# JuliaGaussianProcesses/ApproximateGPs.jl

Measured on AMD Instinct MI355X. Metric: SVGP ELBO evals/sec at N=1e6, M=1024, higher is better.
Workload: dtype f64

## Files before the change

### approximategps.jl_amd/csrc/api.hip

```cpp
#include <hip/hip_runtime.h>

#include <algorithm>
#include <functional>
#include <memory>
#include <cmath>
#include <cstdio>
#include <cstddef>
#include <cstdlib>
#include <cstring>
#include <new>
#include <string>
#include <vector>

#include "../../include/svgp_mi355x.h"
#include "ctx.hpp"
#include "kernels.hpp"
#include "knobs.hpp"
#include "lik.hpp"

using namespace svgp;

inline unsigned event_flags(bool timing) {
  static const bool fence = exp_int("SVGP_EVENT_FENCE", 0) == 1;
  return (timing ? 0u : unsigned(hipEventDisableTiming)) | (fence ? 0u : unsigned(hipEventDisableSystemFence));
// ... 161 lines not shown
KernelParams kparams(const svgp_model* m) {
  KernelParams kp;
  kp.family = m->desc.kernel;
  kp.d = m->d;
  kp.variance = m->desc.variance;
  kp.invl = m->invl.p;
  return kp;
}

inline size_t info_bytes(int64_t Mp) { return (sizeof(int) * size_t(1 + 2 * (Mp / 128)) + 255) / 256 * 256; }
int ensure_overlap(svgp_ctx* ctx, size_t state_doubles);
int enqueue_prep(svgp_ctx* ctx, svgp_model* m, bool overlap = false, const RowHook* hook = nullptr) {
  hipStream_t s = ctx->stream;
  const KernelParams kp = kparams(m);
  HIPC(ctx, hipMemsetAsync(m->info.as<int>(), 0, info_bytes(m->Mp), s));
  launch_scale_inputs(m->dtype, s, m->z_raw.p, m->desc.layout_z, m->d, m->M, m->Mp, m->invl.p, m->zs.p);
  KCHECK(ctx, "scale_inputs");
  if (overlap) {
    launch_pack_q(m->dtype, s, m->Lq_raw.p, m->m_raw.p, m->M, m->Mp, m->U.p, m->mp.p);
    KCHECK(ctx, "pack_q");
    HIPC(ctx, hipEventRecord(ctx->ev_fork, s));
    TREC(ctx, ctx->ev_ov[0], s);
    if (hook && hook->fn) hook->fn(hook->user, -1);
  }
  launch_kuu(m->dtype, s, kp, m->zs.p, m->M, m->Mp, m->desc.jitter, m->L.p);
  KCHECK(ctx, "kuu");
  TREC(ctx, ctx->ev_chol[0], s);
  hipEvent_t rows[16] = {};
  if (overlap) std::copy(std::begin(ctx->ev_row), std::end(ctx->ev_row), rows);
  launch_potrf(m->dtype, s, m->L.p, m->T.p, m->Mp, m->info.as<int>(), reinterpret_cast<unsigned*>(m->info.as<int>() + 1), ctx->num_cus, overlap ? rows : nullptr,
               overlap ? hook : nullptr);
// ... 93 lines not shown
  StripPlan plan = strip_plan(m->dtype, m->Mp, len, ctx->num_cus);
  if (plan.concurrent_tail && (o.A || o.C || o.At || o.Ct)) plan = strip_plan_single(m->dtype, m->Mp, len, ctx->num_cus);
  const size_t wb_main = plan.grid ? strip_work_bytes(m->dtype, m->Mp, plan.nt, plan.grid) : 0;
  const size_t wb_tail = plan.nt_tail ? strip_work_bytes(m->dtype, m->Mp, plan.nt_tail, plan.grid_tail) : 0;
  int rc = ensure_scratch(ctx, plan.concurrent_tail ? wb_main : (wb_main > wb_tail ? wb_main : wb_tail), size_t(len));
  if (rc) return rc;
  if (plan.concurrent_tail) {
    rc = ensure_stream2(ctx);
    if (rc) return rc;
    rc = ctx->work2.reserve(ctx, wb_tail, "the concurrent tail's scratch");
    if (rc) return rc;
  }
  StripArgs a{};
  a.T = m->T.p;
  a.U = m->U.p;
  a.zs = m->zs.p;
  a.mp = m->mp.p;
  a.x = x;
  a.work = ctx->work.p;
  a.counter = ctx->counter.as<unsigned>();
  a.mom_mu = ctx->mom_mu();
  a.mom_var = ctx->mom_var();
  a.A_out = o.A;
  a.C_out = o.C;
  a.At_out = o.At;
  a.Ct_out = o.Ct;
  a.lda = o.lda;
  a.ldx = ldx;
  a.off = off;
  a.len = len;
  a.Mp = m->Mp;
// ... 117 lines not shown

void seg_row_hook(void* user, int row) {
  SegRun& r = *static_cast<SegRun*>(user);
  if (r.rc == SVGP_OK) r.rc = seg_enqueue_row(r, row);
}

int seg_prepare_forward(svgp_ctx* ctx, svgp_model* m, const void* x, int64_t ldx, int64_t off, int64_t len, const OverlapPlan& op, SegRun& r) {
  const int nP = int(m->Mp / 128);
  const size_t wb1 = strip_work_bytes(m->dtype, m->Mp, op.nt, int(op.nstrips)), wb = wb1;
  int rc = ctx->work_seg.reserve(ctx, wb, "the segmented strips' scratch");
  if (rc == SVGP_OK) rc = ensure_scratch(ctx, 0, size_t(len));
  if (rc) return rc;
  r.ctx = ctx; r.m = m; r.op = op; r.grad = false; r.nP = nP; r.wb1 = wb1;
  r.split = seg_split_factor(ctx, nP, op.nstrips);
  StripArgs& a = r.a;
  a.T = m->T.p; a.U = m->U.p; a.zs = m->zs.p; a.mp = m->mp.p; a.x = x; a.work = ctx->work_seg.p; a.counter = ctx->counter2.as<unsigned>();
  a.mom_mu = ctx->mom_mu(); a.mom_var = ctx->mom_var();
  a.ldx = ldx; a.off = off; a.len = len; a.Mp = m->Mp; a.M = m->M; a.kp = kparams(m); a.mean_const = m->desc.mean_const;
  a.seg_state = ctx->seg_state.as<double>();
  return SVGP_OK;
}

int seg_finish_forward(svgp_ctx* ctx, svgp_model* m, const void* y, int64_t off, int64_t len, const StripOuts& o, SegRun& r) {
  hipStream_t s = ctx->stream, s2 = ctx->stream2;
  if (r.rc) return r.rc;
  int launches = r.nP + 1;
  if (r.split > 1) {
    StripArgs& a = r.a;
    const int rcs = seg_split_setup(ctx, a, r.split, r.op.nstrips);
    if (rcs) return rcs;
    a.seg_lo = a.seg_hi = r.nP;
// ... 360 lines not shown
  if (!out) return fail(ctx, SVGP_INVALID_ARG, "null out pointer");
  *out = nullptr;
  int rc = validate_desc(ctx, desc);
  if (rc) return rc;
  HIPC(ctx, hipSetDevice(ctx->device));
  svgp_model* m = new (std::nothrow) svgp_model();
  if (!m) return SVGP_OOM;
  m->M = desc->M;
  m->Mp = (desc->M + 127) / 128 * 128;
  m->dtype = desc->dtype;
  m->d = desc->d;
  m->es = esize(desc->dtype);
  const size_t es = m->es, M = size_t(m->M), Mp = size_t(m->Mp);
  struct { DevBuf* b; size_t bytes; } allocs[] = {
      {&m->z_raw, M * m->d * es}, {&m->m_raw, M * es},     {&m->Lq_raw, M * M * es}, {&m->invl, size_t(m->d) * es},
      {&m->zs, Mp * m->d * es},   {&m->L, Mp * Mp * es},   {&m->T, Mp * Mp * es},    {&m->U, Mp * Mp * es},
      {&m->mp, Mp * es},          {&m->scal, (8 + Mp) * sizeof(double)},             {&m->info, info_bytes(Mp)},
      {&m->B, desc->parametrization == SVGP_CENTERED ? Mp * Mp * es : 0},
  };
  for (auto& a : allocs)
    if (a.bytes && a.b->alloc(a.bytes) != hipSuccess) {
      svgp_model_free(ctx, m);
      return alloc_failed(ctx, "for model buffers");
    }
  if (hipMemsetAsync(m->T.p, 0, Mp * Mp * es, ctx->stream) != hipSuccess) {
    svgp_model_free(ctx, m);
    return fail(ctx, SVGP_HIP_ERROR, "hipMemsetAsync failed for the model's T buffer");
  }
  rc = upload_params(ctx, m, desc);
  if (rc) {
    svgp_model_free(ctx, m);
    return rc;
// ... 110 lines not shown
  if (rc == SVGP_OK) rc = svgp_elbo(ctx, m, D, 0, n, num_data, elbo_out, terms_out);
  else if (ctx->comm) rc = elbo_collective(ctx, rc);
  svgp_data_free(ctx, D);
  svgp_model_free(ctx, m);
  return rc;
}

int32_t svgp_kuf(svgp_ctx* ctx, svgp_model* m, const svgp_data* data, int64_t off, int64_t len, void* Kuf_out_host) {
  int rc = check_batch(ctx, m, data, off, len, false);
  if (rc) return rc;
  HIPC(ctx, hipSetDevice(ctx->device));
  hipStream_t s = ctx->stream;
  const size_t bytes = size_t(m->M) * size_t(len) * m->es;
  rc = ctx->kuf_buf.reserve(ctx, bytes, "Kuf");
  if (rc) return rc;
  launch_scale_inputs(m->dtype, s, m->z_raw.p, m->desc.layout_z, m->d, m->M, m->Mp, m->invl.p, m->zs.p);
  TREC(ctx, ctx->ev[0], s);
  launch_kuf(m->dtype, s, kparams(m), m->zs.p, m->M, m->Mp, data->x.p, data->ldx, off, len, ctx->kuf_buf.p);
  TREC(ctx, ctx->ev[1], s);
  HIPC(ctx, hipGetLastError());
  if (Kuf_out_host) HIPC(ctx, hipMemcpyAsync(Kuf_out_host, ctx->kuf_buf.p, bytes, hipMemcpyDeviceToHost, s));
  HIPC(ctx, hipStreamSynchronize(s));
  float t = 0;
  (void)elapsed_ms(ctx, &t, ctx->ev[0], ctx->ev[1]);
  ctx->timing = svgp_timing{};
  ctx->timing.ms_kuf = t;
  ctx->timing.ms_total = t;
  return SVGP_OK;
}

int32_t svgp_posterior(svgp_ctx* ctx, svgp_model* m, void* Lk_out, void* alpha_out, void* B_out) {
// ... 299 lines not shown
    if (rc) return rc;
    ext_gmu = ctx->ext_g.as<double>();
    ext_gv = ext_gmu + ctx->ext_g.cap / 16;
    HIPC(ctx, hipMemcpyAsync(ext_gmu, gc.ext_gmu, size_t(len) * 8, hipMemcpyHostToDevice, s));
    HIPC(ctx, hipMemcpyAsync(ext_gv, gc.ext_gv, size_t(len) * 8, hipMemcpyHostToDevice, s));
  }
  const bool uniform_w = m->desc.likelihood == SVGP_LIK_GAUSSIAN && !gc.ext_gmu && m->gh_n == 0 && ctx->kn.syrk_uniform;
  static const int early_knob = exp_int("SVGP_SYRK_EARLY", 1);
  const bool syrk_early = gop.on && uniform_w && early_knob != 0;
  if (syrk_early) {
    rc = w->Gmm.reserve(ctx, size_t(std::min<int64_t>(Mp / 128, w->nslices)) * size_t(Mp) * size_t(Mp) * m->es, "the gradient workspace");
    if (rc) return rc;
  }
  auto strip_args = [&](int64_t c0, int64_t clen, LikParams& lpc) -> StripArgs {
    StripArgs a{};
    a.T = m->T.p; a.U = m->U.p; a.zs = m->zs.p; a.mp = m->mp.p; a.x = data->x.p; a.work = ctx->work.p; a.counter = ctx->counter.as<unsigned>();
    a.At_out = w->At.p; a.ldx = data->ldx; a.off = off + c0; a.len = clen; a.Mp = Mp; a.M = M; a.kp = kp;
    a.mean_const = m->desc.mean_const;
    if (gc.mux) a.mux = static_cast<const char*>(gc.mux) + size_t(c0) * es;
    a.mom_mu = ctx->mom_mu(); a.mom_var = ctx->mom_var();
    a.R = w->Rcm.p; a.alpha = w->alpha.p; a.Pt_out = w->Pt.p;
    lpc = lp;
    if (gc.ext_gmu) { lpc.lik = kLikExternal; lpc.gh_x = ext_gmu + c0; lpc.gh_w = ext_gv + c0; }
    return a;
  };
  const void* Bq = centered ? m->B.p : w->Lqp.p;
  auto grad_pre_chain = [&](hipStream_t st) -> int {
    HIPC(ctx, hipMemsetAsync(w->zero_blk.p, 0, w->zero_b, st));
    launch_setvec_f64(st, w->invl_d.as<double>(), m->invl_host.data(), m->d);
    if (!centered) launch_pad_lower(dt, st, m->Lq_raw.p, M, Mp, w->Lqp.p);
    gemm_mm(ctx, w, dt, st, Bq, Bq, Mp, w->G2.p, kMmXUp | kMmYUp);
// ... 812 lines not shown
    int nt, grid; int64_t nstrips;
    chunk_plan(clen, nt, grid, nstrips);
    wb_max = std::max(wb_max, strip_work_bytes(dt, Mp, nt, grid));
  }
  rc = ensure_scratch(ctx, wb_max, size_t(nc));
  if (rc) return rc;
  double* bpart = c->bpart.as<double>();
  double* spart = c->spart.as<double>();
  double* scal = c->scal.as<double>();
  for (int64_t c0 = 0; c0 < len; c0 += nc) {
    const int64_t clen = (len - c0 < nc) ? len - c0 : nc;
    const int64_t ncp = (clen + 127) / 128 * 128;
    int nt, grid; int64_t nstrips;
    chunk_plan(clen, nt, grid, nstrips);
    StripArgs a{};
    a.T = m->T.p; a.zs = m->zs.p; a.x = data->x.p; a.work = ctx->work.p; a.counter = ctx->counter.as<unsigned>();
    a.At_out = w->At.p; a.ldx = data->ldx; a.off = off + c0; a.len = clen; a.Mp = Mp; a.M = M; a.kp = kparams(m);
    a.mom_var = ctx->mom_var();
    HIPC(ctx, hipMemsetAsync(a.counter, 0, sizeof(unsigned), s));
    launch_trsm_point_major(dt, s, a, nt, grid, nstrips);
    KCHECK(ctx, "strip (phase 1, point-major A)");
    const int64_t n16 = (clen + 15) / 16 * 16;
    if (n16 > clen) HIPC(ctx, hipMemsetAsync(static_cast<char*>(w->At.p) + size_t(clen) * size_t(Mp) * es, 0, size_t(n16 - clen) * size_t(Mp) * es, s));
    const int64_t sl = ((ncp + ns_syrk - 1) / ns_syrk + 15) / 16 * 16;
    launch_syrk_uniform(dt, s, w->At.p, 1.0, 1.0, nullptr, 0.0, 1.0, Mp, n16, sl, ns_syrk, w->G1.p, c0 == 0 ? 1 : 0);
    KCHECK(ctx, "syrk (C = A A')");
    launch_collapsed_reduce(dt, s, w->At.p, data->y.p, a.mom_var, Mp, off + c0, clen, m->desc.mean_const, c0 == 0 ? 1 : 0, bpart, spart);
    KCHECK(ctx, "collapsed reduce (b, rr, t)");
  }
  const double sigma2 = m->desc.lik_sigma2;
  int* info_b = c->info_b.as<int>();
// ... 347 lines not shown
```

### approximategps.jl_amd/csrc/ctx.hpp

```cpp
#pragma once
#include <hip/hip_runtime.h>

#include <cstdlib>
#include <string>
#include <vector>

#include "../../include/svgp_mi355x.h"
#include "knobs.hpp"

namespace svgp {
inline int fail(svgp_ctx* ctx, int code, const std::string& msg);
inline int alloc_failed(svgp_ctx* ctx, const std::string& where);


struct DevBuf {
  void* p = nullptr;
  size_t cap = 0;
  bool own = true;
  DevBuf() = default;
  DevBuf(const DevBuf&) = delete;
  DevBuf& operator=(const DevBuf&) = delete;
  ~DevBuf() { release(); }
  void release() {
    if (p && own) (void)hipFree(p);
// ... 153 lines not shown
struct svgp_data {
  int dtype = 0, d = 0;
  int64_t n = 0, ldx = 0;
  svgp::DevBuf x;
  svgp::DevBuf y;
};

struct svgp_model {
  svgp_model_desc desc{};
  std::vector<double> invl_host;
  int64_t M = 0, Mp = 0;
  int dtype = 0, d = 0;
  size_t es = 8;
  svgp::DevBuf z_raw, m_raw, Lq_raw;
  svgp::DevBuf invl, zs, L, T, U, mp, B;
  svgp::DevBuf scal;
  svgp::DevBuf info;
  svgp::DevBuf gh_x, gh_w;
  int gh_n = 0;
  bool prepared = false;
  svgp::DevBuf mu_z;
  double kl = 0, logdet_kuu = 0;
  int chol_info = 0;
};

struct svgp_group {
  std::vector<svgp_ctx*> ctxs;
  std::string err;
};

// ... 44 lines not shown
```

### approximategps.jl_amd/csrc/kernels.hpp

```cpp
#pragma once
#include <hip/hip_runtime.h>
#include <stdint.h>

namespace svgp {

struct KernelParams {
  int family;
  int d;
  double variance;
  const void* invl;
};

constexpr int kLikExternal = -1;
struct LikParams {
  int lik;
  int gh_n;
  double sigma2;
  double digamma_alpha;
  const double* gh_x;
  const double* gh_w;
  int clamp_neg_var;
  double mean_const;
};

void launch_scale_inputs(int dtype, hipStream_t s, const void* z, int layout, int d, int64_t M, int64_t Mp,
                         const void* invl, void* zs);
void launch_transpose_colvecs(int dtype, hipStream_t s, const void* x_dn, int d, int64_t n, int64_t ldx, void* x_fm);
void launch_kuu(int dtype, hipStream_t s, const KernelParams& kp, const void* zs, int64_t M, int64_t Mp,
                double jitter, void* Kuu);
struct RowHook { void (*fn)(void* user, int row) = nullptr; void* user = nullptr; };
void launch_potrf(int dtype, hipStream_t s, void* A, void* T, int64_t Mp, int* info, unsigned* sync, int num_cus, hipEvent_t* row_events = nullptr,
                  const RowHook* hook = nullptr);
int potrf_max_row_events();
void launch_pack_q(int dtype, hipStream_t s, const void* Lq, const void* m, int64_t M, int64_t Mp, void* U, void* mp);
void launch_kl_terms(int dtype, hipStream_t s, const void* Lq, const void* m, const void* Lk, int64_t M, int64_t Mp,
                     double* scal);
void launch_pack_q_ld(int dtype, hipStream_t s, const void* Lq, int64_t ldq, const void* m, int64_t M, int64_t Mp, void* U,
                       void* mp);
void launch_kl_terms_ld(int dtype, hipStream_t s, const void* Lq, int64_t ldq, const void* m, const void* Lk, int64_t M,
                        int64_t Mp, double* scal);
void launch_trsv2(int dtype, hipStream_t s, const void* L, const void* Tm, int64_t Mp, int trans, void* x);
void launch_trsm_mat(int dtype, hipStream_t s, const void* Tm, int64_t Mp, void* X);
void launch_pad_lower(int dtype, hipStream_t s, const void* Lq, int64_t M, int64_t Mp, void* out);
void launch_shift_vec(int dtype, hipStream_t s, const void* m, double shift, int64_t M, int64_t Mp, void* out);
void launch_shift_sub_vec(int dtype, hipStream_t s, const void* m, double shift, const void* mu, int64_t M, int64_t Mp, void* out);
void launch_extract_lower(int dtype, hipStream_t s, const void* A, int64_t Mp, int64_t M, void* out);

enum : int { kSegPregen = 1, kSegPhase2 = 2, kSegLoad = 4, kSegStore = 8 };
struct StripArgs {
  const void* T;
  const void* U;
  const void* zs;
  const void* mp;
  const void* x;
  unsigned* counter;
  void* work;
  double* mom_mu;
  double* mom_var;
  void* A_out;
  void* C_out;
  void* At_out;
  void* Ct_out;
  int64_t lda;
  int64_t ldx, off, len;
  int64_t Mp, M;
  KernelParams kp;
  double mean_const;
// ... 109 lines not shown
```

### approximategps.jl_amd/csrc/prep.hip

```cpp
#define SVGP_DIAG_TU_PREP
#include "device_common.hpp"
#include "kernels.hpp"
#include "knobs.hpp"

#include <hip/hip_ext.h>
#include <cstdlib>
#include <algorithm>
#include <cmath>
#include <map>
#include <mutex>
#include <vector>

namespace svgp {
namespace {

template <typename T>
__global__ void scale_inputs_kernel(const T* __restrict__ z, int layout, int d, int64_t M, int64_t Mp,
                                    const T* __restrict__ invl, T* __restrict__ zs) {
  const int64_t i = int64_t(blockIdx.x) * blockDim.x + threadIdx.x;
  const int f = blockIdx.y;
  if (i >= Mp) return;
  T v = T(0);
  if (i < M) v = (layout == 1 ? z[int64_t(f) * M + i] : z[i * d + f]) * invl[f];
  zs[int64_t(f) * Mp + i] = v;
}

template <typename T>
__global__ void transpose_colvecs_kernel(const T* __restrict__ x, int d, int64_t n, int64_t ldx, T* __restrict__ out) {
  const int64_t i = int64_t(blockIdx.x) * blockDim.x + threadIdx.x;
  if (i >= n) return;
  for (int f = 0; f < d; ++f) out[int64_t(f) * ldx + i] = x[i * d + f];
}

template <typename T, int DREG>
__global__ void __launch_bounds__(k256) kuu_kernel(KernelParams kp, const T* __restrict__ zs, int64_t M, int64_t Mp, T jitter,
                                                   T* __restrict__ K) {
  constexpr int JB = 16;
  const int64_t i = int64_t(blockIdx.x) * k256 + threadIdx.x;
  const int64_t j0 = int64_t(blockIdx.y) * JB;
// ... 820 lines not shown
    hipLaunchKernelGGL((chol_tile_kernel<T, MODE_TRSM, CNT>), dim3((nP * (nP - 1) / 2) * NCH), dim3(k256), lds_tile, s, A, Tm, Mp, -1, 0, info, sync);
    dbg("T panels", s);
  }
}

}

std::string take_note_text() { return take_note(); }

#define SVGP_DISPATCH(dtype, expr_d, expr_f) \
  do {                                       \
    if ((dtype) == 0) { expr_d; } else { expr_f; } \
  } while (0)

void launch_scale_inputs(int dtype, hipStream_t s, const void* z, int layout, int d, int64_t M, int64_t Mp,
                         const void* invl, void* zs) {
  dim3 grid((unsigned)((Mp + 255) / 256), (unsigned)d);
  SVGP_DISPATCH(dtype,
                hipLaunchKernelGGL(scale_inputs_kernel<double>, grid, dim3(256), 0, s, (const double*)z, layout, d, M, Mp, (const double*)invl, (double*)zs),
                hipLaunchKernelGGL(scale_inputs_kernel<float>, grid, dim3(256), 0, s, (const float*)z, layout, d, M, Mp, (const float*)invl, (float*)zs));
}

void launch_transpose_colvecs(int dtype, hipStream_t s, const void* x, int d, int64_t n, int64_t ldx, void* out) {
  dim3 grid((unsigned)((n + 255) / 256));
  SVGP_DISPATCH(dtype,
                hipLaunchKernelGGL(transpose_colvecs_kernel<double>, grid, dim3(256), 0, s, (const double*)x, d, n, ldx, (double*)out),
                hipLaunchKernelGGL(transpose_colvecs_kernel<float>, grid, dim3(256), 0, s, (const float*)x, d, n, ldx, (float*)out));
}

void launch_kuu(int dtype, hipStream_t s, const KernelParams& kp, const void* zs, int64_t M, int64_t Mp, double jitter,
                void* Kuu) {
  dim3 grid((unsigned)((Mp + 255) / 256), (unsigned)(Mp / 16));
  if (kp.d <= 8) {
    SVGP_DISPATCH(dtype,
                  hipLaunchKernelGGL((kuu_kernel<double, 8>), grid, dim3(256), 0, s, kp, (const double*)zs, M, Mp, jitter, (double*)Kuu),
// ... 107 lines not shown
```

### approximategps.jl_amd/csrc/strip.hip

```cpp
#define SVGP_DIAG_TU_STRIP
#include "device_common.hpp"
#include "kernels.hpp"
#include "knobs.hpp"
#include "lik.hpp"

#ifndef SVGP_ASYNC
#define SVGP_ASYNC 1
#endif
#ifndef SVGP_TRI
#define SVGP_TRI 3
#endif

#include <cstdlib>
#include <type_traits>

namespace svgp {

namespace {

#ifndef SVGP_PREGEN_EXPTAB
#define SVGP_PREGEN_EXPTAB 1
#endif
template <typename T, int NT, int NTHR, int F, int DL>
__device__ __forceinline__ void pregen_mfma(const T* __restrict__ xs, const T* __restrict__ zs, int d, int64_t Mp, int64_t M,
                                            double variance_d, T* __restrict__ work, const double* __restrict__ exptab = nullptr) {
  constexpr int KS = DL / 4, JT = NT / 16, NW = NTHR / 64;
  constexpr bool XREG = (DL <= 16);
  using M16 = Mfma16<T>;
  using acc_t = typename M16::acc_t;
  const int lane = threadIdx.x & 63, wave = threadIdx.x >> 6, l15 = lane & 15, g = lane >> 4;
  const T variance = T(variance_d);
  const T c1 = (F == KSE) ? T(-0.5) : T(1);
  const T c0 = (F == KSE) ? T(log(variance_d)) : T(0);
  const T ascale = (F == KSE) ? T(1) : T(-2);
  T xb[XREG ? JT : 1][XREG ? KS : 1], xn[JT];
  const T* __restrict__ xl = xs + g * NT + l15;
#pragma unroll
  for (int jt = 0; jt < JT; ++jt) {
    T s = T(0);
// ... 55 lines not shown
#pragma unroll
        for (int r = 0; r < 4; ++r) work[(k0 + M16::row(lane, r)) * NT + jt * 16 + l15] = out[r];
      } else {
#pragma unroll
        for (int r = 0; r < 4; ++r) {
          const int64_t k = k0 + M16::row(lane, r);
          work[k * NT + jt * 16 + l15] = (k < M) ? out[r] : T(0);
        }
        asm volatile("" ::: "memory");
      }
    }
  }
}


template <typename G, typename T, int NT, int NTHR>
__device__ __forceinline__ void store_tile_point_major(const typename G::Acc& acc, T* __restrict__ smem, T* __restrict__ out,
                                                       int64_t c0, int64_t Mp, int row0) {
  constexpr int HC = NT < 64 ? NT : 64, RS = G::NB + (sizeof(T) == 8 ? 4 : 8), VEC = G::VEC, CPR = G::NB / VEC;
  using V = typename G::V;
  static_assert(size_t(HC) * RS * sizeof(T) <= ((SVGP_ASYNC && G::kAsync) ? G::ASYNC_LDS_BYTES : G::LDS_BYTES),
                "the transposition tile must fit the staging buffers");
#pragma unroll
  for (int p = 0; p < NT / HC; ++p) {
#pragma unroll
    for (int j = 0; j < G::NJ; ++j) {
      const int col = G::acc_col(j);
      if (col / HC == p) {
#pragma unroll
        for (int i = 0; i < G::MI; ++i)
// ... 37 lines not shown
__global__ void __launch_bounds__(NTHR, MINW) strip_kernel(StripArgs a, int64_t nstrips) {
  using G = TileGemm<T, NT, BK, NTHR, PAD>;
  using Acc = typename G::Acc;
  using QRegs = typename G::QRegs;
  constexpr int NB = G::NB, MI = G::MI, NJ = G::NJ, VEC = G::VEC;

  extern __shared__ __attribute__((aligned(16))) unsigned char smem_raw[];
  T* smem = reinterpret_cast<T*>(smem_raw);
  T* xs = smem;
  const int pre_dl = BIGD ? (a.kp.d <= 32 ? 32 : 64) : (a.kp.d <= 8 ? 8 : a.kp.d <= 16 ? 16 : 0);
  const int dl = pre_dl ? pre_dl : a.kp.d;

  const T* __restrict__ Tm = static_cast<const T*>(a.T);
  const T* __restrict__ U = static_cast<const T*>(a.U);
  const T* __restrict__ zs = static_cast<const T*>(a.zs);
  const T* __restrict__ mp = static_cast<const T*>(a.mp);
  const T* __restrict__ x = static_cast<const T*>(a.x);
  const T* __restrict__ invl = static_cast<const T*>(a.kp.invl);
  const int64_t Mp = a.Mp, M = a.M;
  const int d = a.kp.d, family = a.kp.family;
  const T variance = T(a.kp.variance);
  const int nP = int(Mp / NB);
  T* __restrict__ work = static_cast<T*>(a.work) + int64_t(blockIdx.x) * Mp * NT;
  T* __restrict__ workK = (GRAD && !diag::ablate<256>) ? static_cast<T*>(a.work) + (int64_t(gridDim.x) + blockIdx.x) * Mp * NT : work;
  const int tid = threadIdx.x, lane = tid & 63;
  const typename G::QOff qoff = G::q_offsets(NT);

  __shared__ unsigned next_strip;
#if SVGP_PREGEN_EXPTAB
  __shared__ double s_exptab[64];
// ... 45 lines not shown
            const V xf = *reinterpret_cast<const V*>(xs + f * NT + c);
#pragma unroll
            for (int q = 0; q < VEC; ++q) {
              const T df = xf[q] - zf;
              r2[q] = fma(df, df, r2[q]);
            }
          }
          V out;
#pragma unroll
          for (int q = 0; q < VEC; ++q) out[q] = (k < M) ? kappa<T>(F, r2[q], variance) : T(0);
          *reinterpret_cast<V*>(workK + int64_t(k) * NT + c) = out;
        }
      };
      if constexpr (BIGD) {
        if (pre_dl == 32) {
          if (family == KSE) pregen_mfma<T, NT, NTHR, KSE, 32>(xs, zs, d, Mp, M, a.kp.variance, workK, exptab);
          else if (family == KM32) pregen_mfma<T, NT, NTHR, KM32, 32>(xs, zs, d, Mp, M, a.kp.variance, workK);
          else pregen_mfma<T, NT, NTHR, KM52, 32>(xs, zs, d, Mp, M, a.kp.variance, workK);
        } else {
          if (family == KSE) pregen_mfma<T, NT, NTHR, KSE, 64>(xs, zs, d, Mp, M, a.kp.variance, workK, exptab);
          else if (family == KM32) pregen_mfma<T, NT, NTHR, KM32, 64>(xs, zs, d, Mp, M, a.kp.variance, workK);
          else pregen_mfma<T, NT, NTHR, KM52, 64>(xs, zs, d, Mp, M, a.kp.variance, workK);
        }
      } else if (pre_dl == 8) {
        if (family == KSE) pregen_mfma<T, NT, NTHR, KSE, 8>(xs, zs, d, Mp, M, a.kp.variance, workK, exptab);
        else if (family == KM32) pregen_mfma<T, NT, NTHR, KM32, 8>(xs, zs, d, Mp, M, a.kp.variance, workK);
        else pregen_mfma<T, NT, NTHR, KM52, 8>(xs, zs, d, Mp, M, a.kp.variance, workK);
      } else if (pre_dl == 16) {
        if (family == KSE) pregen_mfma<T, NT, NTHR, KSE, 16>(xs, zs, d, Mp, M, a.kp.variance, workK, exptab);
        else if (family == KM32) pregen_mfma<T, NT, NTHR, KM32, 16>(xs, zs, d, Mp, M, a.kp.variance, workK);
        else pregen_mfma<T, NT, NTHR, KM52, 16>(xs, zs, d, Mp, M, a.kp.variance, workK);
      } else if (family == KSE) pregen(std::integral_constant<int, KSE>{});
      else if (family == KM32) pregen(std::integral_constant<int, KM32>{});
      else pregen(std::integral_constant<int, KM52>{});
      __syncthreads();
    }

    double sA[NJ], sM[NJ], sC[NJ];
#pragma unroll
    for (int j = 0; j < NJ; ++j) sA[j] = sM[j] = sC[j] = 0.0;
    int I_lo = 0, I_hi = nP;
    if constexpr (SEG) {
      I_lo = a.seg_lo;
      I_hi = a.seg_hi;
      if ((a.seg_flags & kSegLoad) && part == 0) {
        const double* __restrict__ st = a.seg_state + (strip * NTHR + tid) * (2 * NJ);
// ... 208 lines not shown
}

template <typename T, int NT, int BK, int NTHR, int MINW = 2, int PAD = 16, bool BIGD = false>
__global__ void __launch_bounds__(NTHR, MINW) trsm_pm_kernel(StripArgs a, int64_t nstrips) {
  using G = TileGemm<T, NT, BK, NTHR, PAD>;
  using Acc = typename G::Acc;
  using QRegs = typename G::QRegs;
  constexpr int NB = G::NB, MI = G::MI, NJ = G::NJ;

  extern __shared__ __attribute__((aligned(16))) unsigned char smem_raw[];
  T* smem = reinterpret_cast<T*>(smem_raw);
  T* xs = smem;
  const int pre_dl = BIGD ? (a.kp.d <= 32 ? 32 : 64) : (a.kp.d <= 8 ? 8 : 16);
  const T* __restrict__ Tm = static_cast<const T*>(a.T);
  const T* __restrict__ zs = static_cast<const T*>(a.zs);
  const T* __restrict__ x = static_cast<const T*>(a.x);
  const T* __restrict__ invl = static_cast<const T*>(a.kp.invl);
  const int64_t Mp = a.Mp, M = a.M;
  const int d = a.kp.d, family = a.kp.family;
  const int nP = int(Mp / NB);
  T* __restrict__ work = static_cast<T*>(a.work) + int64_t(blockIdx.x) * Mp * NT;
  const int tid = threadIdx.x, lane = tid & 63;
  [[maybe_unused]] const typename G::QOff qoff = G::q_offsets(NT);

  __shared__ unsigned next_strip;
#if SVGP_PREGEN_EXPTAB
  __shared__ double s_exptab[64];
  if (sizeof(T) == 8 && threadIdx.x < 64) s_exptab[threadIdx.x] = exp2(double(threadIdx.x) * 0.015625);
  const double* exptab = s_exptab;
#else
  const double* exptab = nullptr;
#endif
  for (int64_t strip = blockIdx.x; strip < nstrips;) {
    const int64_t c0 = strip * NT;
    if (tid == 0) next_strip = gridDim.x + atomicAdd(a.counter, 1u);
    const int64_t last = a.off + a.len - 1;
    for (int e = tid; e < pre_dl * NT; e += NTHR) {
      const int f = e / NT, c = e % NT;
      int64_t g = a.off + c0 + c;
      g = g > last ? last : g;
      xs[e] = (f < d) ? x[int64_t(f) * a.ldx + g] * invl[f] : T(0);
    }
    __syncthreads();
    if constexpr (BIGD) {
      if (pre_dl == 32) {
        if (family == KSE) pregen_mfma<T, NT, NTHR, KSE, 32>(xs, zs, d, Mp, M, a.kp.variance, work, exptab);
        else if (family == KM32) pregen_mfma<T, NT, NTHR, KM32, 32>(xs, zs, d, Mp, M, a.kp.variance, work);
        else pregen_mfma<T, NT, NTHR, KM52, 32>(xs, zs, d, Mp, M, a.kp.variance, work);
      } else {
        if (family == KSE) pregen_mfma<T, NT, NTHR, KSE, 64>(xs, zs, d, Mp, M, a.kp.variance, work, exptab);
        else if (family == KM32) pregen_mfma<T, NT, NTHR, KM32, 64>(xs, zs, d, Mp, M, a.kp.variance, work);
        else pregen_mfma<T, NT, NTHR, KM52, 64>(xs, zs, d, Mp, M, a.kp.variance, work);
      }
    } else if (pre_dl == 8) {
      if (family == KSE) pregen_mfma<T, NT, NTHR, KSE, 8>(xs, zs, d, Mp, M, a.kp.variance, work, exptab);
      else if (family == KM32) pregen_mfma<T, NT, NTHR, KM32, 8>(xs, zs, d, Mp, M, a.kp.variance, work);
      else pregen_mfma<T, NT, NTHR, KM52, 8>(xs, zs, d, Mp, M, a.kp.variance, work);
    } else {
      if (family == KSE) pregen_mfma<T, NT, NTHR, KSE, 16>(xs, zs, d, Mp, M, a.kp.variance, work, exptab);
      else if (family == KM32) pregen_mfma<T, NT, NTHR, KM32, 16>(xs, zs, d, Mp, M, a.kp.variance, work);
      else pregen_mfma<T, NT, NTHR, KM52, 16>(xs, zs, d, Mp, M, a.kp.variance, work);
    }
    __syncthreads();

    double sA[NJ];
#pragma unroll
    for (int j = 0; j < NJ; ++j) sA[j] = 0.0;
    for (int I = 0; I < nP; ++I) {
      Acc acc;
      acc.zero();
      if constexpr (SVGP_ASYNC && G::kAsync) {
        auto qsrc = [&](int t) { return work + int64_t(t) * BK * NT; };
        G::template loop_tri_async<(SVGP_TRI & 1) ? 1 : 0>(acc, Tm + int64_t(I) * NB, Mp, (I + 1) * (NB / BK), qsrc, smem);
      } else {
        auto qload = [&](int t, QRegs& r) { G::load_q(r, work + int64_t(t) * BK * NT, qoff); };
        G::template loop_tri<(BK == 16 && (SVGP_TRI & 1)) ? 1 : 0>(acc, Tm + int64_t(I) * NB, Mp, (I + 1) * (NB / BK), qload, smem);
// ... 676 lines not shown
```

Measured before the change: 30.80.

## Precompute inducing-point squared norms and fold norms into MFMA accumulator init

```diff
diff --git a/approximategps.jl_amd/csrc/api.hip b/approximategps.jl_amd/csrc/api.hip
--- a/approximategps.jl_amd/csrc/api.hip
+++ b/approximategps.jl_amd/csrc/api.hip
@@ -199,7 +199,7 @@
   hipStream_t s = ctx->stream;
   const KernelParams kp = kparams(m);
   HIPC(ctx, hipMemsetAsync(m->info.as<int>(), 0, info_bytes(m->Mp), s));
-  launch_scale_inputs(m->dtype, s, m->z_raw.p, m->desc.layout_z, m->d, m->M, m->Mp, m->invl.p, m->zs.p);
+  launch_scale_inputs(m->dtype, s, m->z_raw.p, m->desc.layout_z, m->d, m->M, m->Mp, m->invl.p, m->zs.p, m->znorm.p);
   KCHECK(ctx, "scale_inputs");
   if (overlap) {
     launch_pack_q(m->dtype, s, m->Lq_raw.p, m->m_raw.p, m->M, m->Mp, m->U.p, m->mp.p);
@@ -323,7 +323,7 @@
   StripArgs a{};
   a.T = m->T.p;
   a.U = m->U.p;
-  a.zs = m->zs.p;
+  a.zs = m->zs.p; a.znorm = m->znorm.p;
   a.mp = m->mp.p;
   a.x = x;
   a.work = ctx->work.p;
@@ -471,7 +471,7 @@
   r.ctx = ctx; r.m = m; r.op = op; r.grad = false; r.nP = nP; r.wb1 = wb1;
   r.split = seg_split_factor(ctx, nP, op.nstrips);
   StripArgs& a = r.a;
-  a.T = m->T.p; a.U = m->U.p; a.zs = m->zs.p; a.mp = m->mp.p; a.x = x; a.work = ctx->work_seg.p; a.counter = ctx->counter2.as<unsigned>();
+  a.T = m->T.p; a.U = m->U.p; a.zs = m->zs.p; a.znorm = m->znorm.p; a.mp = m->mp.p; a.x = x; a.work = ctx->work_seg.p; a.counter = ctx->counter2.as<unsigned>();
   a.mom_mu = ctx->mom_mu(); a.mom_var = ctx->mom_var();
   a.ldx = ldx; a.off = off; a.len = len; a.Mp = m->Mp; a.M = m->M; a.kp = kparams(m); a.mean_const = m->desc.mean_const;
   a.seg_state = ctx->seg_state.as<double>();
@@ -862,8 +862,8 @@
   const size_t es = m->es, M = size_t(m->M), Mp = size_t(m->Mp);
   struct { DevBuf* b; size_t bytes; } allocs[] = {
       {&m->z_raw, M * m->d * es}, {&m->m_raw, M * es},     {&m->Lq_raw, M * M * es}, {&m->invl, size_t(m->d) * es},
-      {&m->zs, Mp * m->d * es},   {&m->L, Mp * Mp * es},   {&m->T, Mp * Mp * es},    {&m->U, Mp * Mp * es},
-      {&m->mp, Mp * es},          {&m->scal, (8 + Mp) * sizeof(double)},             {&m->info, info_bytes(Mp)},
+      {&m->zs, Mp * size_t(strip_pad_d(m->d)) * es},   {&m->L, Mp * Mp * es},   {&m->T, Mp * Mp * es},    {&m->U, Mp * Mp * es},
+      {&m->mp, Mp * es},          {&m->znorm, Mp * es},       {&m->scal, (8 + Mp) * sizeof(double)},             {&m->info, info_bytes(Mp)},
       {&m->B, desc->parametrization == SVGP_CENTERED ? Mp * Mp * es : 0},
   };
   for (auto& a : allocs)
@@ -1004,7 +1004,7 @@
   const size_t bytes = size_t(m->M) * size_t(len) * m->es;
   rc = ctx->kuf_buf.reserve(ctx, bytes, "Kuf");
   if (rc) return rc;
-  launch_scale_inputs(m->dtype, s, m->z_raw.p, m->desc.layout_z, m->d, m->M, m->Mp, m->invl.p, m->zs.p);
+  launch_scale_inputs(m->dtype, s, m->z_raw.p, m->desc.layout_z, m->d, m->M, m->Mp, m->invl.p, m->zs.p, m->znorm.p);
   TREC(ctx, ctx->ev[0], s);
   launch_kuf(m->dtype, s, kparams(m), m->zs.p, m->M, m->Mp, data->x.p, data->ldx, off, len, ctx->kuf_buf.p);
   TREC(ctx, ctx->ev[1], s);
@@ -1334,7 +1334,7 @@
   }
   auto strip_args = [&](int64_t c0, int64_t clen, LikParams& lpc) -> StripArgs {
     StripArgs a{};
-    a.T = m->T.p; a.U = m->U.p; a.zs = m->zs.p; a.mp = m->mp.p; a.x = data->x.p; a.work = ctx->work.p; a.counter = ctx->counter.as<unsigned>();
+    a.T = m->T.p; a.U = m->U.p; a.zs = m->zs.p; a.znorm = m->znorm.p; a.mp = m->mp.p; a.x = data->x.p; a.work = ctx->work.p; a.counter = ctx->counter.as<unsigned>();
     a.At_out = w->At.p; a.ldx = data->ldx; a.off = off + c0; a.len = clen; a.Mp = Mp; a.M = M; a.kp = kp;
     a.mean_const = m->desc.mean_const;
     if (gc.mux) a.mux = static_cast<const char*>(gc.mux) + size_t(c0) * es;
@@ -2177,7 +2177,7 @@
     int nt, grid; int64_t nstrips;
     chunk_plan(clen, nt, grid, nstrips);
     StripArgs a{};
-    a.T = m->T.p; a.zs = m->zs.p; a.x = data->x.p; a.work = ctx->work.p; a.counter = ctx->counter.as<unsigned>();
+    a.T = m->T.p; a.zs = m->zs.p; a.znorm = m->znorm.p; a.x = data->x.p; a.work = ctx->work.p; a.counter = ctx->counter.as<unsigned>();
     a.At_out = w->At.p; a.ldx = data->ldx; a.off = off + c0; a.len = clen; a.Mp = Mp; a.M = M; a.kp = kparams(m);
     a.mom_var = ctx->mom_var();
     HIPC(ctx, hipMemsetAsync(a.counter, 0, sizeof(unsigned), s));
diff --git a/approximategps.jl_amd/csrc/ctx.hpp b/approximategps.jl_amd/csrc/ctx.hpp
--- a/approximategps.jl_amd/csrc/ctx.hpp
+++ b/approximategps.jl_amd/csrc/ctx.hpp
@@ -191,6 +191,7 @@
   size_t es = 8;
   svgp::DevBuf z_raw, m_raw, Lq_raw;
   svgp::DevBuf invl, zs, L, T, U, mp, B;
+  svgp::DevBuf znorm;
   svgp::DevBuf scal;
   svgp::DevBuf info;
   svgp::DevBuf gh_x, gh_w;
diff --git a/approximategps.jl_amd/csrc/kernels.hpp b/approximategps.jl_amd/csrc/kernels.hpp
--- a/approximategps.jl_amd/csrc/kernels.hpp
+++ b/approximategps.jl_amd/csrc/kernels.hpp
@@ -23,8 +23,9 @@
   double mean_const;
 };
 
+inline int strip_pad_d(int d) { return d <= 8 ? 8 : d <= 16 ? 16 : d <= 32 ? 32 : 64; }
 void launch_scale_inputs(int dtype, hipStream_t s, const void* z, int layout, int d, int64_t M, int64_t Mp,
-                         const void* invl, void* zs);
+                         const void* invl, void* zs, void* znorm);
 void launch_transpose_colvecs(int dtype, hipStream_t s, const void* x_dn, int d, int64_t n, int64_t ldx, void* x_fm);
 void launch_kuu(int dtype, hipStream_t s, const KernelParams& kp, const void* zs, int64_t M, int64_t Mp,
                 double jitter, void* Kuu);
@@ -51,6 +52,7 @@
   const void* T;
   const void* U;
   const void* zs;
+  const void* znorm;
   const void* mp;
   const void* x;
   unsigned* counter;
diff --git a/approximategps.jl_amd/csrc/prep.hip b/approximategps.jl_amd/csrc/prep.hip
--- a/approximategps.jl_amd/csrc/prep.hip
+++ b/approximategps.jl_amd/csrc/prep.hip
@@ -15,14 +15,25 @@
 namespace {
 
 template <typename T>
-__global__ void scale_inputs_kernel(const T* __restrict__ z, int layout, int d, int64_t M, int64_t Mp,
-                                    const T* __restrict__ invl, T* __restrict__ zs) {
+__global__ void scale_inputs_kernel(const T* __restrict__ z, int layout, int d, int dpad, int64_t M, int64_t Mp,
+                                    const T* __restrict__ invl, T* __restrict__ zs, T* __restrict__ znorm) {
   const int64_t i = int64_t(blockIdx.x) * blockDim.x + threadIdx.x;
-  const int f = blockIdx.y;
   if (i >= Mp) return;
-  T v = T(0);
-  if (i < M) v = (layout == 1 ? z[int64_t(f) * M + i] : z[i * d + f]) * invl[f];
-  zs[int64_t(f) * Mp + i] = v;
+  T sg[4] = {T(0), T(0), T(0), T(0)};
+  for (int f0 = 0; f0 < d; f0 += 4) {
+#pragma unroll
+    for (int g = 0; g < 4; ++g) {
+      const int f = f0 + g;
+      if (f < d) {
+        T v = T(0);
+        if (i < M) v = (layout == 1 ? z[int64_t(f) * M + i] : z[i * d + f]) * invl[f];
+        zs[int64_t(f) * Mp + i] = v;
+        sg[g] = fma(v, v, sg[g]);
+      }
+    }
+  }
+  znorm[i] = (sg[0] + sg[1]) + (sg[2] + sg[3]);
+  for (int f = d; f < dpad; ++f) zs[int64_t(f) * Mp + i] = T(0);
 }
 
 template <typename T>
@@ -873,11 +884,11 @@
   } while (0)
 
 void launch_scale_inputs(int dtype, hipStream_t s, const void* z, int layout, int d, int64_t M, int64_t Mp,
-                         const void* invl, void* zs) {
-  dim3 grid((unsigned)((Mp + 255) / 256), (unsigned)d);
+                         const void* invl, void* zs, void* znorm) {
+  dim3 grid((unsigned)((Mp + 63) / 64));
   SVGP_DISPATCH(dtype,
-                hipLaunchKernelGGL(scale_inputs_kernel<double>, grid, dim3(256), 0, s, (const double*)z, layout, d, M, Mp, (const double*)invl, (double*)zs),
-                hipLaunchKernelGGL(scale_inputs_kernel<float>, grid, dim3(256), 0, s, (const float*)z, layout, d, M, Mp, (const float*)invl, (float*)zs));
+                hipLaunchKernelGGL(scale_inputs_kernel<double>, grid, dim3(64), 0, s, (const double*)z, layout, d, strip_pad_d(d), M, Mp, (const double*)invl, (double*)zs, (double*)znorm),
+                hipLaunchKernelGGL(scale_inputs_kernel<float>, grid, dim3(64), 0, s, (const float*)z, layout, d, strip_pad_d(d), M, Mp, (const float*)invl, (float*)zs, (float*)znorm));
 }
 
 void launch_transpose_colvecs(int dtype, hipStream_t s, const void* x, int d, int64_t n, int64_t ldx, void* out) {
diff --git a/approximategps.jl_amd/csrc/strip.hip b/approximategps.jl_amd/csrc/strip.hip
--- a/approximategps.jl_amd/csrc/strip.hip
+++ b/approximategps.jl_amd/csrc/strip.hip
@@ -22,7 +22,7 @@
 #define SVGP_PREGEN_EXPTAB 1
 #endif
 template <typename T, int NT, int NTHR, int F, int DL>
-__device__ __forceinline__ void pregen_mfma(const T* __restrict__ xs, const T* __restrict__ zs, int d, int64_t Mp, int64_t M,
+__device__ __forceinline__ void pregen_mfma_v1(const T* __restrict__ xs, const T* __restrict__ zs, int d, int64_t Mp, int64_t M,
                                             double variance_d, T* __restrict__ work, const double* __restrict__ exptab = nullptr) {
   constexpr int KS = DL / 4, JT = NT / 16, NW = NTHR / 64;
   constexpr bool XREG = (DL <= 16);
@@ -108,6 +108,119 @@
 }
 
 
+#ifndef SVGP_PREGEN_V2
+#define SVGP_PREGEN_V2 1
+#endif
+template <typename T, int NT, int NTHR, int F, int DL>
+__device__ __forceinline__ void pregen_mfma(const T* __restrict__ xs, const T* __restrict__ zs, const T* __restrict__ znorm, int d, int64_t Mp,
+                                            int64_t M, double variance_d, T* __restrict__ work, const double* __restrict__ exptab = nullptr) {
+  if constexpr (!SVGP_PREGEN_V2) {
+    pregen_mfma_v1<T, NT, NTHR, F, DL>(xs, zs, d, Mp, M, variance_d, work, exptab);
+    return;
+  }
+  constexpr int KS = DL / 4, JT = NT / 16, NW = NTHR / 64;
+  constexpr bool XREG = (DL <= 16);
+  using M16 = Mfma16<T>;
+  using acc_t = typename M16::acc_t;
+  const int lane = threadIdx.x & 63, l15 = lane & 15, g = lane >> 4;
+  const int wave = __builtin_amdgcn_readfirstlane(int(threadIdx.x >> 6));
+  const T variance = T(variance_d);
+  const T c1 = (F == KSE) ? T(-0.5) : T(1);
+  const T c0 = (F == KSE) ? T(log(variance_d)) : T(0);
+  const T ascale = (F == KSE) ? T(1) : T(-2);
+  T xb[XREG ? JT : 1][XREG ? KS : 1], xn[JT];
+  const T* __restrict__ xl = xs + g * NT + l15;
+#pragma unroll
+  for (int jt = 0; jt < JT; ++jt) {
+    T s = T(0);
+#pragma unroll
+    for (int q = 0; q < KS; ++q) {
+      const T v = xl[(4 * q) * NT + jt * 16];
+      if constexpr (XREG) xb[jt][q] = v;
+      s = fma(v, v, s);
+    }
+    s += __shfl_xor(s, 16);
+    s += __shfl_xor(s, 32);
+    xn[jt] = fma(c1, s, c0);
+  }
+  const int nblk = int(Mp / 16);
+  const int zlane = g * int(Mp) + l15;
+  const int wlane = M16::row(lane, 0) * NT + l15;
+  auto zload = [&](int kb, T (&zr)[KS], T (&zq)[4]) {
+    const T* __restrict__ zb = zs + int64_t(kb) * 16;
+    const T* __restrict__ nb = znorm + int64_t(kb) * 16;
+#pragma unroll
+    for (int q = 0; q < KS; ++q) zr[q] = zb[int64_t(4 * q) * Mp + zlane];
+#pragma unroll
+    for (int r = 0; r < 4; ++r) zq[r] = nb[M16::row(lane, r)];
+  };
+  constexpr bool AHEAD = XREG && JT <= 4;
+  T zr[KS], zq[4];
+  if (AHEAD && wave < nblk) zload(wave, zr, zq);
+  for (int kb = wave; kb < nblk; kb += NW) {
+    if constexpr (!AHEAD) zload(kb, zr, zq);
+    const int64_t k0 = int64_t(kb) * 16;
+    const int lim = int(M) - kb * 16;
+    const bool inside = lim >= 16;
+    T za[KS], zn[4];
+#pragma unroll
+    for (int q = 0; q < KS; ++q) za[q] = ascale * zr[q];
+#pragma unroll
+    for (int r = 0; r < 4; ++r) zn[r] = c1 * zq[r];
+    if (AHEAD && kb + NW < nblk) zload(kb + NW, zr, zq);
+    constexpr int IG = (XREG && JT <= 4) ? JT : 1;
+    acc_t accs[IG];
+    T* __restrict__ wp = work + k0 * NT + wlane;
+#pragma unroll
+    for (int jt = 0; jt < JT; ++jt) {
+      acc_t acc;
+      if constexpr (XREG) {
+        if (jt % IG == 0) {
+#pragma unroll
+          for (int t = 0; t < IG; ++t)
+#pragma unroll
+            for (int r = 0; r < 4; ++r) accs[t][r] = xn[jt + t] + zn[r];
+#pragma unroll
+          for (int q = 0; q < KS; ++q)
+#pragma unroll
+            for (int t = 0; t < IG; ++t) accs[t] = M16::mma(za[q], xb[jt + t][q], accs[t]);
+        }
+        acc = accs[jt % IG];
+      } else {
+#pragma unroll
+        for (int r = 0; r < 4; ++r) acc[r] = xn[jt] + zn[r];
+        acc_t acc2 = {0, 0, 0, 0};
+        __builtin_amdgcn_sched_barrier(0);
+#pragma unroll
+        for (int q = 0; q < KS; q += 2) {
+          acc = M16::mma(za[q], xl[(4 * q) * NT + jt * 16], acc);
+          acc2 = M16::mma(za[q + 1], xl[(4 * q + 4) * NT + jt * 16], acc2);
+        }
+#pragma unroll
+        for (int r = 0; r < 4; ++r) acc[r] += acc2[r];
+      }
+      T out[4];
+#pragma unroll
+      for (int r = 0; r < 4; ++r) {
+        const T v = acc[r];
+        if constexpr (SVGP_PREGEN_EXPTAB && F == KSE && sizeof(T) == 8) out[r] = T(kexp_tab(double(v > c0 ? c0 : v), exptab));
+        else out[r] = (F == KSE) ? kexp(v > c0 ? c0 : v) : kappa<T>(F, v < T(0) ? T(0) : v, variance);
+      }
+      if (inside) {
+#pragma unroll
+        for (int r = 0; r < 4; ++r) wp[(M16::row(0, r) - M16::row(0, 0)) * NT + jt * 16] = out[r];
+      } else {
+        int lim_here = lim;
+        asm volatile("" : "+s"(lim_here));
+#pragma unroll
+        for (int r = 0; r < 4; ++r) wp[(M16::row(0, r) - M16::row(0, 0)) * NT + jt * 16] = (M16::row(lane, r) < lim_here) ? out[r] : T(0);
+        asm volatile("" ::: "memory");
+      }
+    }
+  }
+}
+
+
 template <typename G, typename T, int NT, int NTHR>
 __device__ __forceinline__ void store_tile_point_major(const typename G::Acc& acc, T* __restrict__ smem, T* __restrict__ out,
                                                        int64_t c0, int64_t Mp, int row0) {
@@ -175,6 +288,7 @@
   const T* __restrict__ Tm = static_cast<const T*>(a.T);
   const T* __restrict__ U = static_cast<const T*>(a.U);
   const T* __restrict__ zs = static_cast<const T*>(a.zs);
+  const T* __restrict__ znorm = static_cast<const T*>(a.znorm);
   const T* __restrict__ mp = static_cast<const T*>(a.mp);
   const T* __restrict__ x = static_cast<const T*>(a.x);
   const T* __restrict__ invl = static_cast<const T*>(a.kp.invl);
@@ -250,22 +364,22 @@
       };
       if constexpr (BIGD) {
         if (pre_dl == 32) {
-          if (family == KSE) pregen_mfma<T, NT, NTHR, KSE, 32>(xs, zs, d, Mp, M, a.kp.variance, workK, exptab);
-          else if (family == KM32) pregen_mfma<T, NT, NTHR, KM32, 32>(xs, zs, d, Mp, M, a.kp.variance, workK);
-          else pregen_mfma<T, NT, NTHR, KM52, 32>(xs, zs, d, Mp, M, a.kp.variance, workK);
+          if (family == KSE) pregen_mfma<T, NT, NTHR, KSE, 32>(xs, zs, znorm, d, Mp, M, a.kp.variance, workK, exptab);
+          else if (family == KM32) pregen_mfma<T, NT, NTHR, KM32, 32>(xs, zs, znorm, d, Mp, M, a.kp.variance, workK);
+          else pregen_mfma<T, NT, NTHR, KM52, 32>(xs, zs, znorm, d, Mp, M, a.kp.variance, workK);
         } else {
-          if (family == KSE) pregen_mfma<T, NT, NTHR, KSE, 64>(xs, zs, d, Mp, M, a.kp.variance, workK, exptab);
-          else if (family == KM32) pregen_mfma<T, NT, NTHR, KM32, 64>(xs, zs, d, Mp, M, a.kp.variance, workK);
-          else pregen_mfma<T, NT, NTHR, KM52, 64>(xs, zs, d, Mp, M, a.kp.variance, workK);
+          if (family == KSE) pregen_mfma<T, NT, NTHR, KSE, 64>(xs, zs, znorm, d, Mp, M, a.kp.variance, workK, exptab);
+          else if (family == KM32) pregen_mfma<T, NT, NTHR, KM32, 64>(xs, zs, znorm, d, Mp, M, a.kp.variance, workK);
+          else pregen_mfma<T, NT, NTHR, KM52, 64>(xs, zs, znorm, d, Mp, M, a.kp.variance, workK);
         }
       } else if (pre_dl == 8) {
-        if (family == KSE) pregen_mfma<T, NT, NTHR, KSE, 8>(xs, zs, d, Mp, M, a.kp.variance, workK, exptab);
-        else if (family == KM32) pregen_mfma<T, NT, NTHR, KM32, 8>(xs, zs, d, Mp, M, a.kp.variance, workK);
-        else pregen_mfma<T, NT, NTHR, KM52, 8>(xs, zs, d, Mp, M, a.kp.variance, workK);
+        if (family == KSE) pregen_mfma<T, NT, NTHR, KSE, 8>(xs, zs, znorm, d, Mp, M, a.kp.variance, workK, exptab);
+        else if (family == KM32) pregen_mfma<T, NT, NTHR, KM32, 8>(xs, zs, znorm, d, Mp, M, a.kp.variance, workK);
+        else pregen_mfma<T, NT, NTHR, KM52, 8>(xs, zs, znorm, d, Mp, M, a.kp.variance, workK);
       } else if (pre_dl == 16) {
-        if (family == KSE) pregen_mfma<T, NT, NTHR, KSE, 16>(xs, zs, d, Mp, M, a.kp.variance, workK, exptab);
-        else if (family == KM32) pregen_mfma<T, NT, NTHR, KM32, 16>(xs, zs, d, Mp, M, a.kp.variance, workK);
-        else pregen_mfma<T, NT, NTHR, KM52, 16>(xs, zs, d, Mp, M, a.kp.variance, workK);
+        if (family == KSE) pregen_mfma<T, NT, NTHR, KSE, 16>(xs, zs, znorm, d, Mp, M, a.kp.variance, workK, exptab);
+        else if (family == KM32) pregen_mfma<T, NT, NTHR, KM32, 16>(xs, zs, znorm, d, Mp, M, a.kp.variance, workK);
+        else pregen_mfma<T, NT, NTHR, KM52, 16>(xs, zs, znorm, d, Mp, M, a.kp.variance, workK);
       } else if (family == KSE) pregen(std::integral_constant<int, KSE>{});
       else if (family == KM32) pregen(std::integral_constant<int, KM32>{});
       else pregen(std::integral_constant<int, KM52>{});
@@ -504,6 +618,7 @@
   const int pre_dl = BIGD ? (a.kp.d <= 32 ? 32 : 64) : (a.kp.d <= 8 ? 8 : 16);
   const T* __restrict__ Tm = static_cast<const T*>(a.T);
   const T* __restrict__ zs = static_cast<const T*>(a.zs);
+  const T* __restrict__ znorm = static_cast<const T*>(a.znorm);
   const T* __restrict__ x = static_cast<const T*>(a.x);
   const T* __restrict__ invl = static_cast<const T*>(a.kp.invl);
   const int64_t Mp = a.Mp, M = a.M;
@@ -534,22 +649,22 @@
     __syncthreads();
     if constexpr (BIGD) {
       if (pre_dl == 32) {
-        if (family == KSE) pregen_mfma<T, NT, NTHR, KSE, 32>(xs, zs, d, Mp, M, a.kp.variance, work, exptab);
-        else if (family == KM32) pregen_mfma<T, NT, NTHR, KM32, 32>(xs, zs, d, Mp, M, a.kp.variance, work);
-        else pregen_mfma<T, NT, NTHR, KM52, 32>(xs, zs, d, Mp, M, a.kp.variance, work);
+        if (family == KSE) pregen_mfma<T, NT, NTHR, KSE, 32>(xs, zs, znorm, d, Mp, M, a.kp.variance, work, exptab);
+        else if (family == KM32) pregen_mfma<T, NT, NTHR, KM32, 32>(xs, zs, znorm, d, Mp, M, a.kp.variance, work);
+        else pregen_mfma<T, NT, NTHR, KM52, 32>(xs, zs, znorm, d, Mp, M, a.kp.variance, work);
       } else {
-        if (family == KSE) pregen_mfma<T, NT, NTHR, KSE, 64>(xs, zs, d, Mp, M, a.kp.variance, work, exptab);
-        else if (family == KM32) pregen_mfma<T, NT, NTHR, KM32, 64>(xs, zs, d, Mp, M, a.kp.variance, work);
-        else pregen_mfma<T, NT, NTHR, KM52, 64>(xs, zs, d, Mp, M, a.kp.variance, work);
+        if (family == KSE) pregen_mfma<T, NT, NTHR, KSE, 64>(xs, zs, znorm, d, Mp, M, a.kp.variance, work, exptab);
+        else if (family == KM32) pregen_mfma<T, NT, NTHR, KM32, 64>(xs, zs, znorm, d, Mp, M, a.kp.variance, work);
+        else pregen_mfma<T, NT, NTHR, KM52, 64>(xs, zs, znorm, d, Mp, M, a.kp.variance, work);
       }
     } else if (pre_dl == 8) {
-      if (family == KSE) pregen_mfma<T, NT, NTHR, KSE, 8>(xs, zs, d, Mp, M, a.kp.variance, work, exptab);
-      else if (family == KM32) pregen_mfma<T, NT, NTHR, KM32, 8>(xs, zs, d, Mp, M, a.kp.variance, work);
-      else pregen_mfma<T, NT, NTHR, KM52, 8>(xs, zs, d, Mp, M, a.kp.variance, work);
+      if (family == KSE) pregen_mfma<T, NT, NTHR, KSE, 8>(xs, zs, znorm, d, Mp, M, a.kp.variance, work, exptab);
+      else if (family == KM32) pregen_mfma<T, NT, NTHR, KM32, 8>(xs, zs, znorm, d, Mp, M, a.kp.variance, work);
+      else pregen_mfma<T, NT, NTHR, KM52, 8>(xs, zs, znorm, d, Mp, M, a.kp.variance, work);
     } else {
-      if (family == KSE) pregen_mfma<T, NT, NTHR, KSE, 16>(xs, zs, d, Mp, M, a.kp.variance, work, exptab);
-      else if (family == KM32) pregen_mfma<T, NT, NTHR, KM32, 16>(xs, zs, d, Mp, M, a.kp.variance, work);
-      else pregen_mfma<T, NT, NTHR, KM52, 16>(xs, zs, d, Mp, M, a.kp.variance, work);
+      if (family == KSE) pregen_mfma<T, NT, NTHR, KSE, 16>(xs, zs, znorm, d, Mp, M, a.kp.variance, work, exptab);
+      else if (family == KM32) pregen_mfma<T, NT, NTHR, KM32, 16>(xs, zs, znorm, d, Mp, M, a.kp.variance, work);
+      else pregen_mfma<T, NT, NTHR, KM52, 16>(xs, zs, znorm, d, Mp, M, a.kp.variance, work);
     }
     __syncthreads();
 
```

Result: no change. 30.92, median of 6 (+0.4%).
